# ur-whitelab/hoomd-tf

Hardware: AMD Instinct MI355X
Metric: MD steps/sec + achieved HBM GB/s, 131072 particles NN=128 (131k-particle box of the BASELINE metric) (higher is better)
Workload: dtype f32

## Files before the change

### hoomd_tf_amd/csrc/standin.hip

```cpp
#include <cstdlib>
#include <unordered_map>

#include "htf_common.h"
#include "box_math.h"
#include "htf_standin.h"
#include "standin_gate.h"
#include "key_sort.h"

namespace htf {

thread_local Gate g_gate = {nullptr, 0.f};

template <typename T>
__global__ __launch_bounds__(256) void nve_step_kernel(typename Vec4<T>::type *__restrict__ pos,
                                                       typename Vec4<T>::type *__restrict__ vel,
                                                       const typename Vec4<T>::type *__restrict__ force,
                                                       unsigned N, T dt, SBox<T> b) {
    unsigned i = blockIdx.x * blockDim.x + threadIdx.x;
    if (i >= N) return;
    auto p = pos[i];
    auto v = vel[i];
    nve_advance<T>(p, v, force[i], dt, b);
    pos[i] = p;
    vel[i] = v;
// ... 62 lines not shown
    for (unsigned m = 0; m < mirror.n; ++m) {
        const unsigned *src = (const unsigned *)mirror.src[m];
        unsigned *dst = (unsigned *)mirror.dst[m];
        for (unsigned w = threadIdx.x; w < mirror.words[m]; w += blockDim.x) dst[w] = __builtin_nontemporal_load(src + w);
    }
    __threadfence_system();
    __syncthreads();
    if (threadIdx.x == 0) {
        const float worst = __uint_as_float(atomicExch(work, 0u));
        const unsigned cycle = __float_as_uint(out[1]) + 1u;
        out[0] = worst;
        out[1] = __uint_as_float(cycle);
        work[1] = 0u;
        if (h_out != nullptr) {
            h_out[0] = worst;
            __threadfence_system();
            *(volatile unsigned *)(h_out + 1) = cycle;
        }
    }
}

template <typename T>
__device__ __forceinline__ int cell_coord(T x, T lo, T Linv, int n) {
    int c = (int)floor((x - lo) * Linv * (T)n);
    return c < 0 ? 0 : (c >= n ? n - 1 : c);
}

template <typename T>
__global__ __launch_bounds__(256) void cell_index_kernel(const typename Vec4<T>::type *__restrict__ pos, unsigned Ntot,
                                                         SBox<T> b, int nx, int ny, int nz,
                                                         unsigned *__restrict__ cell_of, Gate gate) {
    if (gate.closed()) return;
    unsigned i = blockIdx.x * blockDim.x + threadIdx.x;
    if (i >= Ntot) return;
    auto p = pos[i];
    if (is_inert(p.x)) {
        cell_of[i] = kDeadCell;
        return;
    }
    int cx = cell_coord<T>(p.x, b.lo[0], b.Linv[0], nx);
    int cy = cell_coord<T>(p.y, b.lo[1], b.Linv[1], ny);
    int cz = cell_coord<T>(p.z, b.lo[2], b.Linv[2], nz);
    cell_of[i] = (unsigned)((cz * ny + cy) * nx + cx);
}

constexpr unsigned kTagSide = 1u << 31;
constexpr unsigned kRangeWrapShift = 28u, kRangeLenMask = (1u << kRangeWrapShift) - 1u;
struct RangesArgs {
    int nx, ny, nz, wx, wy, wz, px, py, pz;
    const unsigned *cell_start;
    uint4 *table;
    unsigned *max_neigh;
};
__device__ __forceinline__ void cell_ranges_body(const unsigned t, const RangesArgs &a) {
    const int nx = a.nx, ny = a.ny, nz = a.nz, wx = a.wx, wy = a.wy, wz = a.wz, px = a.px, py = a.py, pz = a.pz;
    const unsigned *__restrict__ cell_start = a.cell_start;
    uint4 *__restrict__ table = a.table;
    unsigned *__restrict__ max_neigh = a.max_neigh;
    const int nrow = (2 * wy + 1) * (2 * wz + 1);
    if (t == 0) *max_neigh = 0u;
    const unsigned ncell = (unsigned)(nx * ny * nz);
    if (t >= ncell * (unsigned)nrow) return;
    const int c = (int)(t / nrow), r = (int)(t % nrow);
    const int cx = c % nx, cy = (c / nx) % ny, cz = c / (nx * ny);
    const int dz = r / (2 * wy + 1) - wz, dy = r % (2 * wy + 1) - wy;
    int a0 = cx - wx, a1 = cx + wx, b0 = 0, b1 = -1;
    if (a0 < 0) {
        if (px) { b0 = nx + a0; b1 = nx - 1; }
        a0 = 0;
    } else if (a1 >= nx) {
        if (px) { b0 = 0; b1 = a1 - nx; }
        a1 = nx - 1;
    }
    int ay = cy + dy, az = cz + dz;
    bool skip = false;
    unsigned wrap_y = 0u, wrap_z = 0u;
    if (ay < 0) { skip |= !py; ay += ny; wrap_y = 1u; } else if (ay >= ny) { skip |= !py; ay -= ny; wrap_y = 2u; }
    if (az < 0) { skip |= !pz; az += nz; wrap_z = 1u; } else if (az >= nz) { skip |= !pz; az -= nz; wrap_z = 2u; }
    uint4 o = make_uint4(0u, 0u, 0u, 0u);
    if (!skip) {
        const unsigned rowbase = (unsigned)((az * ny + ay) * nx);
        o.x = cell_start[rowbase + a0];
        o.y = (cell_start[rowbase + a1 + 1] - o.x) | (wrap_y << kRangeWrapShift) | (wrap_z << (kRangeWrapShift + 2));
        if (b1 >= b0) {
            o.z = cell_start[rowbase + b0];
            o.w = (cell_start[rowbase + b1 + 1] - o.z) | ((b0 == 0 ? 2u : 1u) << kRangeWrapShift);
        }
    }
    table[t] = o;
}
__global__ __launch_bounds__(256) void cell_ranges_kernel(RangesArgs a, Gate gate) {
    if (gate.closed()) return;
    cell_ranges_body(blockIdx.x * blockDim.x + threadIdx.x, a);
}

template <typename T, int G, bool SHIFT>
__global__ __launch_bounds__(256) void build_nlist_kernel(const typename Vec4<T>::type *__restrict__ pos,
                                                          const typename Vec4<T>::type *__restrict__ pos_sorted,
                                                          unsigned N, SBox<T> b, T rl2, int nx, int ny, int nz,
                                                          int wx, int wy, int wz,
                                                          const unsigned *__restrict__ cell_start, unsigned pitch,
                                                          int type_split,
                                                          unsigned *__restrict__ n_neigh, unsigned *__restrict__ head_list,
                                                          unsigned *__restrict__ nlist, unsigned *__restrict__ max_neigh,
                                                          const uint4 *__restrict__ ranges, Gate gate) {
    if (gate.closed()) return;
    const unsigned lane = threadIdx.x & 63u, g = lane % G, sub = lane / G;
    const unsigned i = ((blockIdx.x * blockDim.x + threadIdx.x) >> 6) * (64 / G) + sub;
    const bool in_range = i < N;
    const auto pi = pos[in_range ? i : 0];
    const bool active = in_range && !is_inert(pi.x);
    const int cx = cell_coord<T>(pi.x, b.lo[0], b.Linv[0], nx);
    const int cy = cell_coord<T>(pi.y, b.lo[1], b.Linv[1], ny);
    const int cz = cell_coord<T>(pi.z, b.lo[2], b.Linv[2], nz);
    const bool side_i = type_split >= 0 && scalar_as_int(pi.w) >= type_split;
    unsigned count = 0;
    unsigned *row = nlist + (size_t)(active ? i : 0) * pitch;
    const int nrow = (2 * wy + 1) * (2 * wz + 1);
    const uint4 *mine = ranges + (size_t)((cz * ny + cy) * nx + cx) * nrow;
    uint4 rg_next = active ? mine[0] : make_uint4(0u, 0u, 0u, 0u);
    for (int r = 0; r < nrow; ++r) {
        const uint4 rg = rg_next;
        if (r + 1 < nrow) rg_next = active ? mine[r + 1] : make_uint4(0u, 0u, 0u, 0u);
        T piy = pi.y, piz = pi.z, six = (T)0;
        if (SHIFT) {
            const unsigned wy_ = (rg.y >> kRangeWrapShift) & 3u, wz_ = rg.y >> (kRangeWrapShift + 2), wx_ = rg.w >> kRangeWrapShift;
            piy += wy_ == 1u ? b.L[1] : (wy_ == 2u ? -b.L[1] : (T)0);
            piz += wz_ == 1u ? b.L[2] : (wz_ == 2u ? -b.L[2] : (T)0);
            six = wx_ == 1u ? b.L[0] : -b.L[0];
        }
#pragma unroll
        for (int part = 0; part < 2; ++part) {
            const unsigned beg = part ? rg.z : rg.x, len = (part ? rg.w : rg.y) & kRangeLenMask;
            const T pix = (SHIFT && part) ? pi.x + six : pi.x;
// ... 127 lines not shown
#pragma unroll
            for (unsigned step = 32u; step != 0u; step >>= 1) {
                const unsigned t = at + step;
                at = bperm_u(t, start) <= q ? t : at;
            }
            const bool valid = q < total;
            const unsigned src = bperm_u(at, beg) + (q - bperm_u(at, start));
            V4 pk;
            pk.x = pk.y = pk.z = (T)0;
            set_tag(pk.w, ~0u);
            if (valid) pk = pos_sorted[src];
            if (any_shift) {
                pk.x -= bperm_t(at, shx);
                pk.y -= bperm_t(at, shy);
                pk.z -= bperm_t(at, shz);
            }
            const unsigned tag = (unsigned)scalar_as_int(pk.w);
            const unsigned k = tag & ~kTagSide;
            const unsigned long long vmask = ballot64(valid);
#pragma unroll
            for (int p = 0; p < kCellBatch; ++p) {
                const unsigned i = tag_p[p] & ~kTagSide;
                if (i >= N) continue;
                T ddx = pk.x - px[p], ddy = pk.y - py[p], ddz = pk.z - pz[p];
                if (!SHIFT) {
                    ddx = mimg<T>(ddx, b.L[0], b.Linv[0], b.periodic[0]);
                    ddy = mimg<T>(ddy, b.L[1], b.Linv[1], b.periodic[1]);
                    ddz = mimg<T>(ddz, b.L[2], b.Linv[2], b.periodic[2]);
                }
                unsigned long long hits = vmask & ballot64(k != i) & ballot64(ddx * ddx + ddy * ddy + ddz * ddz <= rl2);
                if (type_split >= 0) {
                    asm volatile("" ::: "memory");
                    hits &= ballot64(((tag ^ tag_p[p]) & kTagSide) == 0u);
                }
                const unsigned rank = __builtin_amdgcn_mbcnt_hi((unsigned)(hits >> 32), __builtin_amdgcn_mbcnt_lo((unsigned)hits, count[p]));
                if (inverse_ballot64(hits) && rank < pitch) nlist[row_p[p] + rank] = k;
                count[p] += (unsigned)__builtin_popcountll(hits);
            }
        }
        unsigned cnt = 0u;
#pragma unroll
        for (int p = 0; p < kCellBatch; ++p) cnt = lane == (unsigned)p ? count[p] : cnt;
        if (lane < np) {
            const unsigned i = my_tag & ~kTagSide;
            if (i < N) {
                n_neigh[i] = cnt < pitch ? cnt : pitch;
                head_list[i] = i * pitch;
                if (cnt > *(volatile unsigned *)max_neigh) atomicMax(max_neigh, cnt);
            }
        }
    }
}

}

using namespace htf;

extern "C" int htfs_nve_step(void *d_pos, void *d_vel, const void *d_force, int dtype, unsigned N, double dt,
                             const htf_box *box, htf_stream stream) {
    HTF_REQUIRE(d_pos && d_vel && d_force && box, "htfs_nve_step: null pointer");
    if (N == 0) return HTF_OK;
    unsigned grid = (N + 255) / 256;
    if (dtype == HTF_F32)
        hipLaunchKernelGGL((nve_step_kernel<float>), dim3(grid), dim3(256), 0, (hipStream_t)stream, (float4 *)d_pos, (float4 *)d_vel, (const float4 *)d_force, N, (float)dt, make_sbox<float>(box));
    else
        hipLaunchKernelGGL((nve_step_kernel<double>), dim3(grid), dim3(256), 0, (hipStream_t)stream, (double4 *)d_pos, (double4 *)d_vel, (const double4 *)d_force, N, dt, make_sbox<double>(box));
    return check_launch("nve_step_kernel");
}

extern "C" int htfs_max_displacement2(const void *d_pos, const void *d_ref, int dtype, unsigned N, const htf_box *box,
                                      float *d_out, htf_stream stream) {
    HTF_REQUIRE(d_pos && d_ref && box && d_out, "htfs_max_displacement2: null pointer");
    if (N == 0) return HTF_OK;
    unsigned grid = (N + 1023) / 1024;
    if (dtype == HTF_F32)
        hipLaunchKernelGGL((max_disp_kernel<float>), dim3(grid), dim3(1024), 0, (hipStream_t)stream, (const float4 *)d_pos, (const float4 *)d_ref, N, make_sbox<float>(box), d_out);
    else
        hipLaunchKernelGGL((max_disp_kernel<double>), dim3(grid), dim3(1024), 0, (hipStream_t)stream, (const double4 *)d_pos, (const double4 *)d_ref, N, make_sbox<double>(box), d_out);
    return check_launch("max_disp_kernel");
}

extern "C" int htfs_check_displacement2(const void *d_pos, const void *d_ref, int dtype, unsigned N, const htf_box *box,
                                        unsigned *d_work, float *d_out, float *h_out, const htfs_mirror *mirror, htf_stream stream) {
    using namespace htf;
    HTF_REQUIRE(d_pos && d_ref && box && d_work && d_out, "htfs_check_displacement2: null pointer");
    HTF_REQUIRE(N > 0, "htfs_check_displacement2: no rows");
    htfs_mirror mr = {};
    if (mirror != nullptr) {
        mr = *mirror;
        HTF_REQUIRE(mr.n <= HTFS_MIRROR_MAX, "htfs_check_displacement2: %u mirrors (at most %d)", mr.n, HTFS_MIRROR_MAX);
        for (unsigned m = 0; m < mr.n; ++m)
            HTF_REQUIRE(mr.src[m] && mr.dst[m] && ((uintptr_t)mr.src[m] & 3) == 0 && ((uintptr_t)mr.dst[m] & 3) == 0,
                        "htfs_check_displacement2: mirror %u: null or unaligned pointer", m);
    }
    unsigned grid = (N + 1023) / 1024;
    if (dtype == HTF_F32)
        hipLaunchKernelGGL((check_disp_kernel<float>), dim3(grid), dim3(1024), 0, (hipStream_t)stream, (const float4 *)d_pos, (const float4 *)d_ref, N, make_sbox<float>(box), d_work, d_out, h_out, mr);
    else
        hipLaunchKernelGGL((check_disp_kernel<double>), dim3(grid), dim3(1024), 0, (hipStream_t)stream, (const double4 *)d_pos, (const double4 *)d_ref, N, make_sbox<double>(box), d_work, d_out, h_out, mr);
    return check_launch("check_disp_kernel");
}

namespace htf {
struct Reimage {
    double L[3], c[3];
};
// ... 89 lines not shown
    for (unsigned i = 0; i < kScanPer; ++i) c[i] = first + i < ncell ? count[first + i] : 0u;
    unsigned sum = 0;
#pragma unroll
    for (unsigned i = 0; i < kScanPer; ++i) sum += c[i];
    unsigned incl = sum;
#pragma unroll
    for (unsigned off = 1; off < 64; off <<= 1) {
        const unsigned v = (unsigned)__shfl_up((int)incl, off);
        if (lane >= off) incl += v;
    }
    if (lane == 63) s_wave[wave] = incl;
    __syncthreads();
    unsigned before = 0, total = 0, carry = 0;
#pragma unroll
    for (unsigned w = 0; w < kScanThreads / 64; ++w) {
        const unsigned v = s_wave[w];
        before += w < wave ? v : 0u;
        total += v;
        carry += s_carry[w];
    }
    unsigned run = carry + before + (incl - sum);
#pragma unroll
    for (unsigned i = 0; i < kScanPer; ++i)
        if (first + i < ncell) {
            start[first + i] = run;
            cursor[first + i] = run;
            run += c[i];
        }
    if (blockIdx.x == gridDim.x - 1 && t == 0) start[ncell] = carry + total;
}

__global__ __launch_bounds__(256) void cell_scatter_kernel(const unsigned *__restrict__ cell_of, unsigned n,
                                                           unsigned *__restrict__ cursor, unsigned *__restrict__ order, Gate gate) {
    if (gate.closed()) return;
    const unsigned i = blockIdx.x * blockDim.x + threadIdx.x;
    if (i < n && cell_of[i] != kDeadCell) order[atomicAdd(&cursor[cell_of[i]], 1u)] = i;
}

__global__ __launch_bounds__(256) void cell_order_kernel(const unsigned *__restrict__ start, unsigned ncell,
                                                         unsigned *__restrict__ order, unsigned *__restrict__ count, Gate gate) {
    if (gate.closed()) return;
    const unsigned c = blockIdx.x * blockDim.x + threadIdx.x;
    if (c >= ncell) return;
    count[c] = 0u;
    const unsigned b = start[c], e = start[c + 1];
    for (unsigned i = b + 1; i < e; ++i) {
        const unsigned v = order[i];
        unsigned j = i;
        while (j > b && order[j - 1] > v) {
            order[j] = order[j - 1];
            --j;
        }
        order[j] = v;
    }
}
}

static int zero_counts_if_needed(unsigned *count, unsigned ncell, hipStream_t s) {
    static thread_local std::unordered_map<const void *, unsigned> zeroed_for;
    HTF_REQUIRE(((uintptr_t)count & 15) == 0, "binning scratch must be 16-byte aligned (cell_scan_kernel reads it with 16-byte loads)");
    auto it = zeroed_for.find(count);
    if (!g_gate.disp2 || it == zeroed_for.end() || it->second != ncell) {
        HTF_CHECK_HIP(hipMemsetAsync(count, 0, (size_t)ncell * sizeof(unsigned), s));
        zeroed_for[count] = ncell;
    }
    return HTF_OK;
}

extern "C" int htfs_cell_sort(const unsigned *d_cell_of, unsigned Ntot, unsigned ncell, unsigned *d_scratch,
                              unsigned *d_cell_start, unsigned *d_order, htf_stream stream) {
    using namespace htf;
    HTF_REQUIRE(d_cell_of && d_scratch && d_cell_start && d_order, "htfs_cell_sort: null pointer");
    HTF_REQUIRE(ncell > 0, "htfs_cell_sort: no cells");
    hipStream_t s = (hipStream_t)stream;
    unsigned *count = d_scratch, *cursor = d_scratch + ncell;
    if (int rc = zero_counts_if_needed(count, ncell, s)) return rc;
    if (Ntot) hipLaunchKernelGGL(cell_count_kernel, dim3((Ntot + 255) / 256), dim3(256), 0, s, d_cell_of, Ntot, count, g_gate);
    hipLaunchKernelGGL(cell_scan_kernel, dim3((ncell + kScanChunk - 1) / kScanChunk), dim3(kScanThreads), 0, s, count, ncell, d_cell_start, cursor, g_gate);
    if (Ntot) hipLaunchKernelGGL(cell_scatter_kernel, dim3((Ntot + 255) / 256), dim3(256), 0, s, d_cell_of, Ntot, cursor, d_order, g_gate);
    hipLaunchKernelGGL(cell_order_kernel, dim3((ncell + 255) / 256), dim3(256), 0, s, d_cell_start, ncell, d_order, count, g_gate);
    return check_launch("htfs_cell_sort");
}

static int gather4(void *d_dest, const void *d_src, const int *d_order, int dtype, unsigned n, bool tag, int type_split,
                   htf_stream stream, const unsigned *d_n_live = nullptr) {
    using namespace htf;
    HTF_REQUIRE(d_dest && d_src && d_order, "htfs_gather4: null pointer");
    HTF_REQUIRE(!tag || n <= kTagSide, "htfs_gather4_tagged: %u particles do not fit the 31-bit tag", n);
    if (n == 0) return HTF_OK;
    const dim3 grid((n + 255) / 256), block(256);
    hipStream_t s = (hipStream_t)stream;
    if (dtype == HTF_F32) {
        if (tag) hipLaunchKernelGGL((gather4_kernel<float4, true>), grid, block, 0, s, (float4 *)d_dest, (const float4 *)d_src, d_order, n, type_split, g_gate, d_n_live);
        else hipLaunchKernelGGL((gather4_kernel<float4, false>), grid, block, 0, s, (float4 *)d_dest, (const float4 *)d_src, d_order, n, type_split, g_gate, d_n_live);
    } else {
        if (tag) hipLaunchKernelGGL((gather4_kernel<double4, true>), grid, block, 0, s, (double4 *)d_dest, (const double4 *)d_src, d_order, n, type_split, g_gate, d_n_live);
        else hipLaunchKernelGGL((gather4_kernel<double4, false>), grid, block, 0, s, (double4 *)d_dest, (const double4 *)d_src, d_order, n, type_split, g_gate, d_n_live);
    }
    return check_launch("gather4_kernel");
}

extern "C" int htfs_gather4(void *d_dest, const void *d_src, const int *d_order, int dtype, unsigned n, htf_stream stream) {
    return gather4(d_dest, d_src, d_order, dtype, n, false, -1, stream);
}

extern "C" int htfs_gather4_tagged(void *d_dest, const void *d_src, const int *d_order, int dtype, unsigned n, int type_split,
// ... 62 lines not shown
#pragma unroll 1
    while (seg + 1 < t.n && row >= t.cnt[seg]) {
        row -= t.cnt[seg];
        ++seg;
    }
    dst[(size_t)(t.dst[seg] + row) * row_words + col] = src[(size_t)(t.src[seg] + row) * row_words + col];
}

extern "C" int htfs_segment_copy(void *d_dst, const void *d_src, unsigned row_bytes, unsigned n_segments,
                                 const unsigned *src_start, const unsigned *dst_start, const unsigned *count, htf_stream stream) {
    HTF_REQUIRE(d_dst && d_src && src_start && dst_start && count, "htfs_segment_copy: null pointer");
    HTF_REQUIRE(n_segments >= 1 && n_segments <= HTFS_MAX_SEGMENTS && row_bytes % 4 == 0 && row_bytes > 0,
                "htfs_segment_copy: need 1..%d segments of whole 32-bit words", HTFS_MAX_SEGMENTS);
    SegTable t;
    t.n = 0;
    unsigned total = 0;
    for (unsigned s = 0; s < n_segments; ++s) {
        if (count[s] == 0) continue;
        t.src[t.n] = src_start[s];
        t.dst[t.n] = dst_start[s];
        t.cnt[t.n] = count[s];
        total += count[s];
        ++t.n;
    }
    if (total == 0) return HTF_OK;
    const unsigned words = row_bytes / 4;
    const unsigned grid = (unsigned)(((size_t)total * words + 255) / 256);
    hipLaunchKernelGGL(segment_copy_kernel, dim3(grid), dim3(256), 0, (hipStream_t)stream, (unsigned *)d_dst, (const unsigned *)d_src,
                       words, t, total);
    return check_launch("segment_copy_kernel");
}

extern "C" int htfs_cell_index(const void *d_pos, int dtype, unsigned Ntot, const htf_box *box, const int *ncell3,
                               unsigned *d_cell_of, htf_stream stream) {
    HTF_REQUIRE(d_pos && box && ncell3 && d_cell_of, "htfs_cell_index: null pointer");
    if (Ntot == 0) return HTF_OK;
    unsigned grid = (Ntot + 255) / 256;
    if (dtype == HTF_F32)
        hipLaunchKernelGGL((cell_index_kernel<float>), dim3(grid), dim3(256), 0, (hipStream_t)stream, (const float4 *)d_pos, Ntot, make_sbox<float>(box), ncell3[0], ncell3[1], ncell3[2], d_cell_of, g_gate);
    else
        hipLaunchKernelGGL((cell_index_kernel<double>), dim3(grid), dim3(256), 0, (hipStream_t)stream, (const double4 *)d_pos, Ntot, make_sbox<double>(box), ncell3[0], ncell3[1], ncell3[2], d_cell_of, g_gate);
    return check_launch("cell_index_kernel");
}

struct FinishArgs {
    void *pos_sorted;
    const int *order;
    unsigned n;
    void *ref;
    unsigned n_ref;
    unsigned *counter;
    htf::Reimage im;
};

static int build_nlist_impl(const void *d_pos, const void *d_pos_sorted, int dtype, unsigned N, unsigned Ntot,
                            const htf_box *box, double r_list, const int *ncell3, const int *stencil3,
                            const unsigned *d_cell_start, unsigned pitch, int type_split,
                            unsigned *d_n_neigh, unsigned *d_head_list, unsigned *d_nlist, unsigned *d_max_neigh,
                            void *d_ranges_v, htf_stream stream, const FinishArgs *fin) {
    (void)Ntot;
    HTF_REQUIRE(d_pos && d_pos_sorted && box && ncell3 && stencil3 && d_cell_start && d_n_neigh && d_head_list && d_nlist && d_max_neigh,
                "htfs_build_nlist: null pointer");
    HTF_REQUIRE(pitch > 0, "htfs_build_nlist: pitch must be > 0");
    for (int d = 0; d < 3; ++d) {
        const double w = (box->hi[d] - box->lo[d]) / ncell3[d];
        const int sw = stencil3[d];
        HTF_REQUIRE((sw == 0 && ncell3[d] == 1) || (sw >= 1 && sw <= 2 && ncell3[d] >= 2 * sw + 1 && w * sw >= r_list * (1.0 - 1e-12)),
                    "htfs_build_nlist: along %d need 1 cell, or >= 2w+1 cells with w cells spanning r_list (got %d cells of %g, stencil %d, r_list %g)",
                    d, ncell3[d], w, sw, r_list);
    }
    if (N == 0) return HTF_OK;
    const unsigned ncell = (unsigned)(ncell3[0] * ncell3[1] * ncell3[2]);
    const unsigned nrow = (unsigned)((2 * stencil3[1] + 1) * (2 * stencil3[2] + 1));
    HTF_REQUIRE(d_ranges_v && ((uintptr_t)d_ranges_v & 15) == 0, "htfs_build_nlist: d_ranges must be a 16-byte aligned table of 4 * ncell * rows words");
    uint4 *d_ranges = (uint4 *)d_ranges_v;
    const RangesArgs ra = {ncell3[0], ncell3[1], ncell3[2], stencil3[0], stencil3[1], stencil3[2], (int)box->periodic[0],
                           (int)box->periodic[1], (int)box->periodic[2], d_cell_start, d_ranges, d_max_neigh};
    const unsigned nb_ranges = (ncell * nrow + 255) / 256;
    if (fin == nullptr) {
        hipLaunchKernelGGL(cell_ranges_kernel, dim3(nb_ranges), dim3(256), 0, (hipStream_t)stream, ra, g_gate);
    } else {
        const unsigned nb = nb_ranges + (fin->n + 255) / 256 + (fin->n == 0 ? 1u : 0u);
        if (dtype == HTF_F32)
            hipLaunchKernelGGL((bins_finish_kernel<float4>), dim3(nb), dim3(256), 0, (hipStream_t)stream, ra, nb_ranges, (float4 *)fin->pos_sorted,
                               (const float4 *)d_pos, fin->order, fin->n, type_split, (float4 *)fin->ref, fin->n_ref, fin->counter, fin->im, g_gate);
        else
            hipLaunchKernelGGL((bins_finish_kernel<double4>), dim3(nb), dim3(256), 0, (hipStream_t)stream, ra, nb_ranges, (double4 *)fin->pos_sorted,
                               (const double4 *)d_pos, fin->order, fin->n, type_split, (double4 *)fin->ref, fin->n_ref, fin->counter, fin->im, g_gate);
    }
    const bool fine = stencil3[0] == 2 || stencil3[1] == 2 || stencil3[2] == 2;
#define HTFS_NL(T, V4, G)                                                                                              \
    if (shift) HTFS_NL_(T, V4, G, true); else HTFS_NL_(T, V4, G, false)
#define HTFS_NL_(T, V4, G, S)                                                                                          \
    hipLaunchKernelGGL((build_nlist_kernel<T, G, S>), dim3((N + 4 * (64 / G) - 1) / (4 * (64 / G))), dim3(256), 0, (hipStream_t)stream, \
                       (const V4 *)d_pos, (const V4 *)d_pos_sorted, N, make_sbox<T>(box), (T)(r_list * r_list), ncell3[0],  \
                       ncell3[1], ncell3[2], stencil3[0], stencil3[1], stencil3[2], d_cell_start, pitch,      \
                       type_split, d_n_neigh, d_head_list, d_nlist, d_max_neigh, (const uint4 *)d_ranges, g_gate)
#define HTFS_NLC(T, V4)                                                                                                \
    if (shift) HTFS_NLC_(T, V4, true); else HTFS_NLC_(T, V4, false)
#define HTFS_NLC_(T, V4, S)                                                                                            \
    hipLaunchKernelGGL((build_nlist_cells_kernel<T, S>), dim3((ncell * cell_split + 3) / 4), dim3(256), 0, (hipStream_t)stream, \
                       (const V4 *)d_pos_sorted, N, make_sbox<T>(box), (T)(r_list * r_list), ncell, (int)nrow, d_cell_start, pitch, \
                       type_split, d_n_neigh, d_head_list, d_nlist, d_max_neigh, (const uint4 *)d_ranges, cell_split, g_gate)
    bool shift = true;
    for (int d = 0; d < 3; ++d) shift = shift && (!box->periodic[d] || ncell3[d] >= 7);
#ifdef HTF_AB_VARIANTS
    static const bool per_particle = std::getenv("HTFS_NLIST_PER_PARTICLE") != nullptr, per_cell = std::getenv("HTFS_NLIST_PER_CELL") != nullptr;
#else
    constexpr bool per_particle = false, per_cell = false;
#endif
    const bool reimaged = fin != nullptr && (fin->im.L[0] > 0.0 || fin->im.L[1] > 0.0 || fin->im.L[2] > 0.0);
    const bool by_cell = per_cell || reimaged || (!per_particle && ncell >= 1024u);
    const unsigned cell_split = ncell <= 12288u ? 2u : 1u;
    if (by_cell) {
        if (dtype == HTF_F32) { HTFS_NLC(float, float4); } else { HTFS_NLC(double, double4); }
    } else if (dtype == HTF_F32) {
        if (fine) { HTFS_NL(float, float4, 8); } else { HTFS_NL(float, float4, 16); }
    } else {
        if (fine) { HTFS_NL(double, double4, 8); } else { HTFS_NL(double, double4, 16); }
    }
#undef HTFS_NL
#undef HTFS_NL_
#undef HTFS_NLC
#undef HTFS_NLC_
    return check_launch("build_nlist_kernel");
}

extern "C" int htfs_build_nlist(const void *d_pos, const void *d_pos_sorted, int dtype, unsigned N, unsigned Ntot,
                                const htf_box *box, double r_list, const int *ncell3, const int *stencil3,
                                const unsigned *d_cell_start, unsigned pitch, int type_split,
                                unsigned *d_n_neigh, unsigned *d_head_list, unsigned *d_nlist, unsigned *d_max_neigh,
                                void *d_ranges, htf_stream stream) {
    return build_nlist_impl(d_pos, d_pos_sorted, dtype, N, Ntot, box, r_list, ncell3, stencil3, d_cell_start, pitch, type_split, d_n_neigh,
                            d_head_list, d_nlist, d_max_neigh, d_ranges, stream, nullptr);
}

static int rebuild_nlist_impl(const void *d_pos, int dtype, unsigned N, unsigned Ntot, const htf_box *box, double r_list, const int *ncell3,
                              const int *stencil3, unsigned *d_cell_of, unsigned *d_scratch, unsigned *d_cell_start,
                              unsigned *d_order, void *d_pos_sorted, unsigned pitch, int type_split, unsigned *d_n_neigh,
                              unsigned *d_head_list, unsigned *d_nlist, unsigned *d_max_neigh, void *d_ref,
                              unsigned *d_counter, void *d_ranges, htf_stream stream, bool scratch_clean = false,
                              const double *image_L = nullptr) {
    using namespace htf;
    HTF_REQUIRE(d_pos && box && ncell3 && stencil3 && d_cell_of && d_scratch && d_cell_start && d_order && d_pos_sorted,
                "htfs_rebuild_nlist: null pointer");
    HTF_REQUIRE(Ntot >= N, "htfs_rebuild_nlist: Ntot %u < N %u", Ntot, N);
    if (N == 0) return HTF_OK;
    const unsigned ncell = (unsigned)(ncell3[0] * ncell3[1] * ncell3[2]);
    HTF_REQUIRE(ncell > 0, "htfs_rebuild_nlist: no cells");
    hipStream_t s = (hipStream_t)stream;
    unsigned *count = d_scratch, *cursor = d_scratch + ncell;
    if (!scratch_clean)
        if (int rc = zero_counts_if_needed(count, ncell, s)) return rc;
    const unsigned grid = (Ntot + 255) / 256;
    Reimage im = {};
    for (int d = 0; d < 3; ++d) {
        im.L[d] = image_L != nullptr && !box->periodic[d] ? image_L[d] : 0.0;
        im.c[d] = 0.5 * (box->lo[d] + box->hi[d]);
        HTF_REQUIRE(im.L[d] == 0.0 || im.L[d] >= box->hi[d] - box->lo[d], "htfs_rebuild_nlist_ghosts: image length %g along axis %d is shorter than the grid", im.L[d], d);
    }
    if (dtype == HTF_F32)
        hipLaunchKernelGGL((cell_index_count_kernel<float>), dim3(grid), dim3(256), 0, s, (const float4 *)d_pos, Ntot, make_sbox<float>(box),
                           ncell3[0], ncell3[1], ncell3[2], d_cell_of, count, im, g_gate);
    else
        hipLaunchKernelGGL((cell_index_count_kernel<double>), dim3(grid), dim3(256), 0, s, (const double4 *)d_pos, Ntot, make_sbox<double>(box),
                           ncell3[0], ncell3[1], ncell3[2], d_cell_of, count, im, g_gate);
    hipLaunchKernelGGL(cell_scan_kernel, dim3((ncell + kScanChunk - 1) / kScanChunk), dim3(kScanThreads), 0, s, count, ncell, d_cell_start, cursor, g_gate);
    hipLaunchKernelGGL(cell_scatter_kernel, dim3(grid), dim3(256), 0, s, d_cell_of, Ntot, cursor, d_order, g_gate);
    hipLaunchKernelGGL(cell_order_kernel, dim3((ncell + 255) / 256), dim3(256), 0, s, d_cell_start, ncell, d_order, count, g_gate);
    const FinishArgs fin = {d_pos_sorted, (const int *)d_order, Ntot, d_ref, N, d_counter, im};
    return build_nlist_impl(d_pos, d_pos_sorted, dtype, N, Ntot, box, r_list, ncell3, stencil3, d_cell_start, pitch, type_split, d_n_neigh,
                            d_head_list, d_nlist, d_max_neigh, d_ranges, stream, &fin);
}

extern "C" int htfs_rebuild_nlist(const void *d_pos, int dtype, unsigned N, const htf_box *box, double r_list, const int *ncell3,
                                  const int *stencil3, unsigned *d_cell_of, unsigned *d_scratch, unsigned *d_cell_start,
                                  unsigned *d_order, void *d_pos_sorted, unsigned pitch, int type_split, unsigned *d_n_neigh,
                                  unsigned *d_head_list, unsigned *d_nlist, unsigned *d_max_neigh, void *d_ref,
                                  unsigned *d_counter, void *d_ranges, htf_stream stream) {
    return rebuild_nlist_impl(d_pos, dtype, N, N, box, r_list, ncell3, stencil3, d_cell_of, d_scratch, d_cell_start, d_order, d_pos_sorted,
                              pitch, type_split, d_n_neigh, d_head_list, d_nlist, d_max_neigh, d_ref, d_counter, d_ranges, stream);
}

extern "C" int htfs_rebuild_nlist_ghosts(const void *d_pos, int dtype, unsigned N, unsigned Ntot, const htf_box *box, double r_list,
                                         const int *ncell3, const int *stencil3, unsigned *d_cell_of, unsigned *d_scratch,
                                         unsigned *d_cell_start, unsigned *d_order, void *d_pos_sorted, unsigned pitch, int type_split,
                                         unsigned *d_n_neigh, unsigned *d_head_list, unsigned *d_nlist, unsigned *d_max_neigh, void *d_ref,
                                         unsigned *d_counter, void *d_ranges, int scratch_clean, const double *image_L, htf_stream stream) {
    return rebuild_nlist_impl(d_pos, dtype, N, Ntot, box, r_list, ncell3, stencil3, d_cell_of, d_scratch, d_cell_start, d_order, d_pos_sorted,
                              pitch, type_split, d_n_neigh, d_head_list, d_nlist, d_max_neigh, d_ref, d_counter, d_ranges, stream,
                              scratch_clean != 0, image_L);
}

extern "C" int htfs_check_rebuild_nlist(const void *d_pos, int dtype, unsigned N, const htf_box *box, double r_list, const int *ncell3,
                                        const int *stencil3, unsigned *d_cell_of, unsigned *d_scratch, unsigned *d_cell_start,
                                        unsigned *d_order, void *d_pos_sorted, unsigned pitch, int type_split, unsigned *d_n_neigh,
                                        unsigned *d_head_list, unsigned *d_nlist, unsigned *d_stat2, void *d_ref, float *d_disp2,
                                        double threshold2, unsigned *h_stat2, void *d_ranges, htf_stream stream) {
    HTF_REQUIRE(d_ref && d_disp2 && d_stat2, "htfs_check_rebuild_nlist: null pointer");
    if (N == 0) return HTF_OK;
    HTF_CHECK_HIP(hipMemsetAsync(d_disp2, 0, sizeof(float), (hipStream_t)stream));
    int rc = htfs_max_displacement2(d_pos, d_ref, dtype, N, box, d_disp2, stream);
    if (rc != HTF_OK) return rc;
    rc = htfs_set_gate(d_disp2, threshold2);
    if (rc != HTF_OK) return rc;
    rc = htfs_rebuild_nlist(d_pos, dtype, N, box, r_list, ncell3, stencil3, d_cell_of, d_scratch, d_cell_start, d_order, d_pos_sorted, pitch,
                            type_split, d_n_neigh, d_head_list, d_nlist, d_stat2, d_ref, d_stat2 + 1, d_ranges, stream);
    (void)htfs_set_gate(nullptr, 0.0);
    if (rc != HTF_OK) return rc;
    if (h_stat2 != nullptr)
        HTF_CHECK_HIP(hipMemcpyAsync(h_stat2, d_stat2, 2 * sizeof(unsigned), hipMemcpyDeviceToHost, (hipStream_t)stream));
    return HTF_OK;
}
// ... 29 lines not shown
```

Baseline: 13460.

## Replace six-kernel neighbor-list rebuild with three-kernel bin-count, place, search pipeline

The rebuild path now bins particles into fixed-capacity per-cell slot arrays using atomics. A single place kernel computes cell starts via a block-local prefix sum, orders each cell's members by rank and writes the sorted, reimaged positions. A new search kernel computes the stencil row ranges inside each wave (prefix sum plus binary search over the rows) instead of reading a precomputed range table. This removes the separate scan, scatter, insertion-sort and ranges kernels and their launches. The cost is a slow fallback scan over all particles when a cell overflows its cap, and reuse of the ranges buffer as slot storage.

```diff
diff --git a/hoomd_tf_amd/csrc/standin.hip b/hoomd_tf_amd/csrc/standin.hip
--- a/hoomd_tf_amd/csrc/standin.hip
+++ b/hoomd_tf_amd/csrc/standin.hip
@@ -138,34 +138,48 @@
     uint4 *table;
     unsigned *max_neigh;
 };
+struct RowSpan {
+    int a0, a1, b0, b1;
+    unsigned rowbase, wrap_y, wrap_z;
+    bool skip;
+};
+__device__ __forceinline__ RowSpan row_span(const RangesArgs &a, int c, int r) {
+    const int nx = a.nx, ny = a.ny, nz = a.nz, wx = a.wx, wy = a.wy, wz = a.wz, px = a.px, py = a.py, pz = a.pz;
+    const int cx = c % nx, cy = (c / nx) % ny, cz = c / (nx * ny);
+    const int dw = 2 * wy + 1, q = (r >= dw) + (r >= 2 * dw) + (r >= 3 * dw) + (r >= 4 * dw);
+    const int dz = q - wz, dy = r - q * dw - wy;
+    RowSpan s;
+    s.a0 = cx - wx, s.a1 = cx + wx, s.b0 = 0, s.b1 = -1;
+    if (s.a0 < 0) {
+        if (px) { s.b0 = nx + s.a0; s.b1 = nx - 1; }
+        s.a0 = 0;
+    } else if (s.a1 >= nx) {
+        if (px) { s.b0 = 0; s.b1 = s.a1 - nx; }
+        s.a1 = nx - 1;
+    }
+    int ay = cy + dy, az = cz + dz;
+    s.skip = false;
+    s.wrap_y = 0u, s.wrap_z = 0u;
+    if (ay < 0) { s.skip |= !py; ay += ny; s.wrap_y = 1u; } else if (ay >= ny) { s.skip |= !py; ay -= ny; s.wrap_y = 2u; }
+    if (az < 0) { s.skip |= !pz; az += nz; s.wrap_z = 1u; } else if (az >= nz) { s.skip |= !pz; az -= nz; s.wrap_z = 2u; }
+    s.rowbase = (unsigned)((az * ny + ay) * nx);
+    return s;
+}
 __device__ __forceinline__ void cell_ranges_body(const unsigned t, const RangesArgs &a) {
-    const int nx = a.nx, ny = a.ny, nz = a.nz, wx = a.wx, wy = a.wy, wz = a.wz, px = a.px, py = a.py, pz = a.pz;
     const unsigned *__restrict__ cell_start = a.cell_start;
     uint4 *__restrict__ table = a.table;
     unsigned *__restrict__ max_neigh = a.max_neigh;
-    const int nrow = (2 * wy + 1) * (2 * wz + 1);
+    const int nrow = (2 * a.wy + 1) * (2 * a.wz + 1);
     if (t == 0) *max_neigh = 0u;
-    const unsigned ncell = (unsigned)(nx * ny * nz);
+    const unsigned ncell = (unsigned)(a.nx * a.ny * a.nz);
     if (t >= ncell * (unsigned)nrow) return;
     const int c = (int)(t / nrow), r = (int)(t % nrow);
-    const int cx = c % nx, cy = (c / nx) % ny, cz = c / (nx * ny);
-    const int dz = r / (2 * wy + 1) - wz, dy = r % (2 * wy + 1) - wy;
-    int a0 = cx - wx, a1 = cx + wx, b0 = 0, b1 = -1;
-    if (a0 < 0) {
-        if (px) { b0 = nx + a0; b1 = nx - 1; }
-        a0 = 0;
-    } else if (a1 >= nx) {
-        if (px) { b0 = 0; b1 = a1 - nx; }
-        a1 = nx - 1;
-    }
-    int ay = cy + dy, az = cz + dz;
-    bool skip = false;
-    unsigned wrap_y = 0u, wrap_z = 0u;
-    if (ay < 0) { skip |= !py; ay += ny; wrap_y = 1u; } else if (ay >= ny) { skip |= !py; ay -= ny; wrap_y = 2u; }
-    if (az < 0) { skip |= !pz; az += nz; wrap_z = 1u; } else if (az >= nz) { skip |= !pz; az -= nz; wrap_z = 2u; }
+    const RowSpan s = row_span(a, c, r);
+    const int a0 = s.a0, a1 = s.a1, b0 = s.b0, b1 = s.b1;
+    const unsigned wrap_y = s.wrap_y, wrap_z = s.wrap_z;
     uint4 o = make_uint4(0u, 0u, 0u, 0u);
-    if (!skip) {
-        const unsigned rowbase = (unsigned)((az * ny + ay) * nx);
+    if (!s.skip) {
+        const unsigned rowbase = s.rowbase;
         o.x = cell_start[rowbase + a0];
         o.y = (cell_start[rowbase + a1 + 1] - o.x) | (wrap_y << kRangeWrapShift) | (wrap_z << (kRangeWrapShift + 2));
         if (b1 >= b0) {
@@ -399,6 +413,148 @@
     }
 }
 
+constexpr int kSearchTripsDefault = 1;
+template <typename T, bool SHIFT, int kSearchTrips>
+__global__ __launch_bounds__(256) void search_cells_kernel(const typename Vec4<T>::type *__restrict__ pos_sorted, unsigned N, SBox<T> b,
+                                                           T rl2, RangesArgs ra, unsigned pitch, int type_split,
+                                                           unsigned *__restrict__ n_neigh, unsigned *__restrict__ head_list,
+                                                           unsigned *__restrict__ nlist, unsigned *__restrict__ max_neigh, unsigned split,
+                                                           unsigned *__restrict__ bin_count, Gate gate) {
+    if (gate.closed()) return;
+    using V4 = typename Vec4<T>::type;
+    const unsigned lane = threadIdx.x & 63u;
+    const unsigned *__restrict__ cell_start = ra.cell_start;
+    const unsigned ncell = (unsigned)(ra.nx * ra.ny * ra.nz);
+    const int nrow = (2 * ra.wy + 1) * (2 * ra.wz + 1);
+    const unsigned wv = __builtin_amdgcn_readfirstlane((blockIdx.x * blockDim.x + threadIdx.x) >> 6);
+    const unsigned c = wv / split, b0 = wv % split;
+    if (c >= ncell) return;
+    if (b0 == 0u && lane == 0u) bin_count[c] = 0u;
+    const unsigned p_begin = cell_start[c], p_end = cell_start[c + 1];
+    if (p_begin + b0 * (unsigned)kCellBatch >= p_end) return;
+
+    unsigned beg = 0u, len = 0u;
+    T shx = (T)0, shy = (T)0, shz = (T)0;
+    if (lane < 2u * (unsigned)nrow) {
+        const RowSpan s = row_span(ra, (int)c, (int)(lane >> 1));
+        const bool wrapped = (lane & 1u) != 0u;
+        const int lo = wrapped ? s.b0 : s.a0, hi = wrapped ? s.b1 : s.a1;
+        if (!s.skip && hi >= lo) {
+            beg = cell_start[s.rowbase + lo];
+            len = cell_start[s.rowbase + hi + 1] - beg;
+        }
+        if (SHIFT) {
+            shy = s.wrap_y == 1u ? b.L[1] : (s.wrap_y == 2u ? -b.L[1] : (T)0);
+            shz = s.wrap_z == 1u ? b.L[2] : (s.wrap_z == 2u ? -b.L[2] : (T)0);
+            shx = !wrapped ? (T)0 : (s.b0 == 0 ? -b.L[0] : b.L[0]);
+        }
+    }
+    if (p_end - p_begin <= 64u) {
+        const bool local = lane < p_end - p_begin && ((unsigned)scalar_as_int(pos_sorted[p_begin + lane].w) & ~kTagSide) < N;
+        if (ballot64(local) == 0ull) return;
+    }
+    unsigned incl = len;
+#pragma unroll
+    for (unsigned d = 1; d < 64u; d <<= 1) {
+        const unsigned up = bperm_u(lane >= d ? lane - d : lane, incl);
+        incl += lane >= d ? up : 0u;
+    }
+    const unsigned start = incl - len;
+    const unsigned total = (unsigned)__builtin_amdgcn_readlane((int)incl, 63);
+    const bool any_shift = SHIFT && ballot64(len != 0u && (shx != (T)0 || shy != (T)0 || shz != (T)0)) != 0ull;
+
+    for (unsigned pb = p_begin + b0 * (unsigned)kCellBatch; pb < p_end; pb += split * (unsigned)kCellBatch) {
+        const unsigned np = min(p_end - pb, (unsigned)kCellBatch);
+        V4 me;
+        me.x = me.y = me.z = (T)0;
+        set_tag(me.w, ~0u);
+        if (lane < np) me = pos_sorted[pb + lane];
+        const unsigned my_tag = (unsigned)scalar_as_int(me.w);
+        if (ballot64(lane < np && (my_tag & ~kTagSide) < N) == 0ull) continue;
+        unsigned tag_p[kCellBatch], count[kCellBatch];
+        T px[kCellBatch], py[kCellBatch], pz[kCellBatch];
+        unsigned row_p[kCellBatch];
+#pragma unroll
+        for (int p = 0; p < kCellBatch; ++p) {
+            tag_p[p] = ~0u;
+            px[p] = py[p] = pz[p] = (T)0;
+            count[p] = 0u;
+            row_p[p] = 0u;
+            if ((unsigned)p < np) {
+                tag_p[p] = (unsigned)__builtin_amdgcn_readlane((int)my_tag, p);
+                px[p] = in_vgpr(bcast_lane_t(me.x, p));
+                py[p] = in_vgpr(bcast_lane_t(me.y, p));
+                pz[p] = in_vgpr(bcast_lane_t(me.z, p));
+                row_p[p] = (tag_p[p] & ~kTagSide) * pitch;
+            }
+        }
+        for (unsigned q0 = 0; q0 < total; q0 += 64u * kSearchTrips) {
+            V4 pk[kSearchTrips];
+            unsigned at[kSearchTrips];
+#pragma unroll
+            for (int u = 0; u < kSearchTrips; ++u) {
+                pk[u].x = pk[u].y = pk[u].z = (T)0;
+                set_tag(pk[u].w, ~0u);
+                at[u] = 0u;
+                if (q0 + 64u * u >= total) continue;
+                const unsigned q = q0 + 64u * u + lane;
+                unsigned a_ = 0u;
+#pragma unroll
+                for (unsigned step = 32u; step != 0u; step >>= 1) {
+                    const unsigned t = a_ + step;
+                    a_ = bperm_u(t, start) <= q ? t : a_;
+                }
+                at[u] = a_;
+                const unsigned src = bperm_u(a_, beg) + (q - bperm_u(a_, start));
+                if (q < total) pk[u] = pos_sorted[src];
+            }
+#pragma unroll
+            for (int u = 0; u < kSearchTrips; ++u) {
+                if (q0 + 64u * u >= total) break;
+                V4 cand = pk[u];
+                if (any_shift) {
+                    cand.x -= bperm_t(at[u], shx);
+                    cand.y -= bperm_t(at[u], shy);
+                    cand.z -= bperm_t(at[u], shz);
+                }
+                const unsigned tag = (unsigned)scalar_as_int(cand.w);
+                const unsigned k = tag & ~kTagSide;
+                const unsigned long long vmask = ballot64(q0 + 64u * u + lane < total);
+#pragma unroll
+                for (int p = 0; p < kCellBatch; ++p) {
+                    const unsigned i = tag_p[p] & ~kTagSide;
+                    if (i >= N) continue;
+                    T ddx = cand.x - px[p], ddy = cand.y - py[p], ddz = cand.z - pz[p];
+                    if (!SHIFT) {
+                        ddx = mimg<T>(ddx, b.L[0], b.Linv[0], b.periodic[0]);
+                        ddy = mimg<T>(ddy, b.L[1], b.Linv[1], b.periodic[1]);
+                        ddz = mimg<T>(ddz, b.L[2], b.Linv[2], b.periodic[2]);
+                    }
+                    unsigned long long hits = vmask & ballot64(k != i) & ballot64(ddx * ddx + ddy * ddy + ddz * ddz <= rl2);
+                    if (type_split >= 0) {
+                        asm volatile("" ::: "memory");
+                        hits &= ballot64(((tag ^ tag_p[p]) & kTagSide) == 0u);
+                    }
+                    const unsigned rank = __builtin_amdgcn_mbcnt_hi((unsigned)(hits >> 32), __builtin_amdgcn_mbcnt_lo((unsigned)hits, count[p]));
+                    if (inverse_ballot64(hits) && rank < pitch) nlist[row_p[p] + rank] = k;
+                    count[p] += (unsigned)__builtin_popcountll(hits);
+                }
+            }
+        }
+        unsigned cnt = 0u;
+#pragma unroll
+        for (int p = 0; p < kCellBatch; ++p) cnt = lane == (unsigned)p ? count[p] : cnt;
+        if (lane < np) {
+            const unsigned i = my_tag & ~kTagSide;
+            if (i < N) {
+                n_neigh[i] = cnt < pitch ? cnt : pitch;
+                head_list[i] = i * pitch;
+                if (cnt > *(volatile unsigned *)max_neigh) atomicMax(max_neigh, cnt);
+            }
+        }
+    }
+}
+
 }
 
 using namespace htf;
@@ -594,6 +750,115 @@
             --j;
         }
         order[j] = v;
+    }
+}
+
+constexpr unsigned kBinLanes = 8, kBinCells = 256 / kBinLanes;
+
+template <typename T>
+__global__ __launch_bounds__(256) void bin_count_kernel(const typename Vec4<T>::type *__restrict__ pos, unsigned Ntot, SBox<T> b,
+                                                        int nx, int ny, int nz, unsigned *__restrict__ cell_of,
+                                                        unsigned *__restrict__ count, unsigned *__restrict__ slots, unsigned cap,
+                                                        Reimage im, Gate gate) {
+    if (gate.closed()) return;
+    const unsigned i = blockIdx.x * blockDim.x + threadIdx.x;
+    if (i >= Ntot) return;
+    const auto p = pos[i];
+    if (is_inert(p.x)) {
+        cell_of[i] = kDeadCell;
+        return;
+    }
+    const int cx = cell_coord<T>(reimage1(p.x, im.L[0], im.c[0]), b.lo[0], b.Linv[0], nx);
+    const int cy = cell_coord<T>(reimage1(p.y, im.L[1], im.c[1]), b.lo[1], b.Linv[1], ny);
+    const int cz = cell_coord<T>(reimage1(p.z, im.L[2], im.c[2]), b.lo[2], b.Linv[2], nz);
+    const unsigned c = (unsigned)((cz * ny + cy) * nx + cx);
+    cell_of[i] = c;
+    const unsigned slot = atomicAdd(&count[c], 1u);
+    if (slot < cap) slots[(size_t)c * cap + slot] = i;
+}
+
+template <typename V>
+__global__ __launch_bounds__(256) void bin_place_kernel(unsigned ncell, unsigned Ntot, const unsigned *__restrict__ cell_of,
+                                                        const unsigned *__restrict__ count, const unsigned *__restrict__ slots,
+                                                        unsigned cap, unsigned *__restrict__ cell_start, unsigned *__restrict__ order,
+                                                        V *__restrict__ dest, const V *__restrict__ src, int type_split, V *__restrict__ ref,
+                                                        unsigned n_ref, unsigned *__restrict__ counter, unsigned *__restrict__ max_neigh,
+                                                        Reimage im, Gate gate) {
+    if (gate.closed()) return;
+    __shared__ unsigned s_before[4], s_cnt[kBinCells], s_start[kBinCells];
+    const unsigned t = threadIdx.x, lane = t & 63u, g = t % kBinLanes, cl = t / kBinLanes;
+    const unsigned c = blockIdx.x * kBinCells + cl;
+    unsigned before = 0u;
+    {
+        const uint4 *q = reinterpret_cast<const uint4 *>(count);
+        const unsigned nq = blockIdx.x * (kBinCells / 4u);
+        for (unsigned j0 = 0; j0 < nq; j0 += 8u * blockDim.x) {
+            uint4 v[8];
+#pragma unroll
+            for (unsigned u = 0; u < 8u; ++u) {
+                const unsigned j = j0 + u * blockDim.x + t;
+                v[u] = j < nq ? q[j] : make_uint4(0u, 0u, 0u, 0u);
+            }
+#pragma unroll
+            for (unsigned u = 0; u < 8u; ++u) before += (v[u].x + v[u].y) + (v[u].z + v[u].w);
+        }
+    }
+    before = group_sum_u<64>(before);
+    if (lane == 0u) s_before[t >> 6] = before;
+    const unsigned cnt = c < ncell ? count[c] : 0u;
+    if (g == 0u) s_cnt[cl] = cnt;
+    if (t == 0u && blockIdx.x == 0u) {
+        if (counter != nullptr) *counter += 1u;
+        *max_neigh = 0u;
+    }
+    __syncthreads();
+    if (t < kBinCells) {
+        const unsigned v = s_cnt[t];
+        unsigned incl = v;
+#pragma unroll
+        for (unsigned off = 1; off < kBinCells; off <<= 1) {
+            const unsigned up = (unsigned)__shfl_up((int)incl, off, kBinCells);
+            if (t >= off) incl += up;
+        }
+        const unsigned base = (s_before[0] + s_before[1]) + (s_before[2] + s_before[3]);
+        s_start[t] = base + incl - v;
+        if (t == kBinCells - 1u && blockIdx.x == gridDim.x - 1u) cell_start[ncell] = base + incl;
+    }
+    __syncthreads();
+    const unsigned first = s_start[cl];
+    if (g == 0u && c < ncell) cell_start[c] = first;
+    auto place = [&](unsigned k, unsigned d) {
+        order[d] = k;
+        V p = src[k];
+        if (ref != nullptr && k < n_ref) ref[k] = p;
+        p.x = reimage1(p.x, im.L[0], im.c[0]);
+        p.y = reimage1(p.y, im.L[1], im.c[1]);
+        p.z = reimage1(p.z, im.L[2], im.c[2]);
+        set_tag(p.w, k | ((type_split >= 0 && scalar_as_int(p.w) >= type_split) ? kTagSide : 0u));
+        dest[d] = p;
+    };
+    const bool fits = cnt <= cap;
+    const unsigned *mine = slots + (size_t)(c < ncell ? c : 0u) * cap;
+    for (unsigned k0 = 0; ballot64(fits && k0 < cnt) != 0ull; k0 += kBinLanes) {
+        const bool have = fits && k0 + g < cnt;
+        const unsigned me = have ? mine[k0 + g] : ~0u;
+        unsigned rank = 0u;
+        for (unsigned j0 = 0; ballot64(fits && j0 < cnt) != 0ull; j0 += kBinLanes) {
+            const unsigned o = fits && j0 + g < cnt ? mine[j0 + g] : ~0u;
+#pragma unroll
+            for (unsigned j = 0; j < kBinLanes; ++j) rank += (unsigned)__shfl((int)o, (int)j, (int)kBinLanes) < me ? 1u : 0u;
+        }
+        if (have) place(me, first + rank);
+    }
+    if (ballot64(!fits) != 0ull) {
+        unsigned done = 0u;
+        for (unsigned j0 = 0; j0 < Ntot; j0 += kBinLanes) {
+            const unsigned j = j0 + g;
+            const bool hit = !fits && j < Ntot && cell_of[j] == c;
+            const unsigned m = (unsigned)(ballot64(hit) >> (lane & ~(kBinLanes - 1u))) & ((1u << kBinLanes) - 1u);
+            if (hit) place(j, first + done + (unsigned)__popc(m & ((1u << g) - 1u)));
+            done += (unsigned)__popc(m);
+        }
     }
 }
 }
@@ -762,6 +1027,17 @@
     unsigned *counter;
     htf::Reimage im;
 };
+
+static bool search_by_cell(unsigned ncell, const htf::Reimage *im) {
+#ifdef HTF_AB_VARIANTS
+    static const bool per_particle = std::getenv("HTFS_NLIST_PER_PARTICLE") != nullptr, per_cell = std::getenv("HTFS_NLIST_PER_CELL") != nullptr;
+#else
+    constexpr bool per_particle = false, per_cell = false;
+#endif
+    const bool reimaged = im != nullptr && (im->L[0] > 0.0 || im->L[1] > 0.0 || im->L[2] > 0.0);
+    return per_cell || reimaged || (!per_particle && ncell >= 1024u);
+}
+static unsigned search_cell_split(unsigned ncell) { return ncell <= 12288u ? 2u : 1u; }
 
 static int build_nlist_impl(const void *d_pos, const void *d_pos_sorted, int dtype, unsigned N, unsigned Ntot,
                             const htf_box *box, double r_list, const int *ncell3, const int *stencil3,
@@ -814,14 +1090,8 @@
                        type_split, d_n_neigh, d_head_list, d_nlist, d_max_neigh, (const uint4 *)d_ranges, cell_split, g_gate)
     bool shift = true;
     for (int d = 0; d < 3; ++d) shift = shift && (!box->periodic[d] || ncell3[d] >= 7);
-#ifdef HTF_AB_VARIANTS
-    static const bool per_particle = std::getenv("HTFS_NLIST_PER_PARTICLE") != nullptr, per_cell = std::getenv("HTFS_NLIST_PER_CELL") != nullptr;
-#else
-    constexpr bool per_particle = false, per_cell = false;
-#endif
-    const bool reimaged = fin != nullptr && (fin->im.L[0] > 0.0 || fin->im.L[1] > 0.0 || fin->im.L[2] > 0.0);
-    const bool by_cell = per_cell || reimaged || (!per_particle && ncell >= 1024u);
-    const unsigned cell_split = ncell <= 12288u ? 2u : 1u;
+    const bool by_cell = search_by_cell(ncell, fin != nullptr ? &fin->im : nullptr);
+    const unsigned cell_split = search_cell_split(ncell);
     if (by_cell) {
         if (dtype == HTF_F32) { HTFS_NLC(float, float4); } else { HTFS_NLC(double, double4); }
     } else if (dtype == HTF_F32) {
@@ -869,6 +1139,63 @@
         im.c[d] = 0.5 * (box->lo[d] + box->hi[d]);
         HTF_REQUIRE(im.L[d] == 0.0 || im.L[d] >= box->hi[d] - box->lo[d], "htfs_rebuild_nlist_ghosts: image length %g along axis %d is shorter than the grid", im.L[d], d);
     }
+#ifdef HTF_AB_VARIANTS
+    static const bool three = std::getenv("HTFS_REBUILD_LEGACY") == nullptr;
+#else
+    constexpr bool three = true;
+#endif
+    if (three && ncell >= 2u && search_by_cell(ncell, &im)) {
+        HTF_REQUIRE(d_ranges && ((uintptr_t)d_ranges & 15) == 0 && d_n_neigh && d_head_list && d_nlist && d_max_neigh,
+                    "htfs_rebuild_nlist: null pointer");
+        for (int d = 0; d < 3; ++d) {
+            const double w = (box->hi[d] - box->lo[d]) / ncell3[d];
+            const int sw = stencil3[d];
+            HTF_REQUIRE((sw == 0 && ncell3[d] == 1) || (sw >= 1 && sw <= 2 && ncell3[d] >= 2 * sw + 1 && w * sw >= r_list * (1.0 - 1e-12)),
+                        "htfs_build_nlist: along %d need 1 cell, or >= 2w+1 cells with w cells spanning r_list (got %d cells of %g, stencil %d, r_list %g)",
+                        d, ncell3[d], w, sw, r_list);
+        }
+        HTF_REQUIRE(pitch > 0, "htfs_build_nlist: pitch must be > 0");
+        HTF_REQUIRE(Ntot <= kTagSide, "htfs_rebuild_nlist: %u particles do not fit the 31-bit tag", Ntot);
+        const unsigned nrow = (unsigned)((2 * stencil3[1] + 1) * (2 * stencil3[2] + 1));
+        unsigned *slots = (unsigned *)d_ranges;
+        const unsigned cap = 4u * nrow;
+        const RangesArgs ra = {ncell3[0], ncell3[1], ncell3[2], stencil3[0], stencil3[1], stencil3[2], (int)box->periodic[0],
+                               (int)box->periodic[1], (int)box->periodic[2], d_cell_start, nullptr, d_max_neigh};
+        const dim3 place_grid((ncell + kBinCells - 1) / kBinCells), search_grid((ncell * search_cell_split(ncell) + 3) / 4);
+        bool shift = true;
+        for (int d = 0; d < 3; ++d) shift = shift && (!box->periodic[d] || ncell3[d] >= 7);
+#ifdef HTF_AB_VARIANTS
+        static const int trips = std::getenv("HTFS_SEARCH_TRIPS") != nullptr ? std::atoi(std::getenv("HTFS_SEARCH_TRIPS")) : kSearchTripsDefault;
+#else
+        constexpr int trips = kSearchTripsDefault;
+#endif
+#define HTFS_SEARCH3(T, V4, S, U)                                                                                                     \
+    hipLaunchKernelGGL((search_cells_kernel<T, S, U>), search_grid, dim3(256), 0, s, (const V4 *)d_pos_sorted, N, make_sbox<T>(box),  \
+                       (T)(r_list * r_list), ra, pitch, type_split, d_n_neigh, d_head_list, d_nlist, d_max_neigh,                     \
+                       search_cell_split(ncell), count, g_gate)
+#define HTFS_REBUILD3(T, V4)                                                                                                          \
+    do {                                                                                                                              \
+        hipLaunchKernelGGL((bin_count_kernel<T>), dim3(grid), dim3(256), 0, s, (const V4 *)d_pos, Ntot, make_sbox<T>(box), ncell3[0],  \
+                           ncell3[1], ncell3[2], d_cell_of, count, slots, cap, im, g_gate);                                           \
+        hipLaunchKernelGGL((bin_place_kernel<V4>), place_grid, dim3(256), 0, s, ncell, Ntot, d_cell_of, count, slots, cap,            \
+                           d_cell_start, d_order, (V4 *)d_pos_sorted, (const V4 *)d_pos, type_split, (V4 *)d_ref, N, d_counter,       \
+                           d_max_neigh, im, g_gate);                                                                                  \
+        if (shift) {                                                                                                                  \
+            if (trips == 1) HTFS_SEARCH3(T, V4, true, 1);                                                                             \
+            else if (trips == 2) HTFS_SEARCH3(T, V4, true, 2);                                                                        \
+            else HTFS_SEARCH3(T, V4, true, 4);                                                                                        \
+        } else {                                                                                                                      \
+            if (trips == 1) HTFS_SEARCH3(T, V4, false, 1);                                                                            \
+            else if (trips == 2) HTFS_SEARCH3(T, V4, false, 2);                                                                       \
+            else HTFS_SEARCH3(T, V4, false, 4);                                                                                       \
+        }                                                                                                                             \
+    } while (0)
+        if (dtype == HTF_F32) HTFS_REBUILD3(float, float4);
+        else HTFS_REBUILD3(double, double4);
+#undef HTFS_SEARCH3
+#undef HTFS_REBUILD3
+        return check_launch("htfs_rebuild_nlist");
+    }
     if (dtype == HTF_F32)
         hipLaunchKernelGGL((cell_index_count_kernel<float>), dim3(grid), dim3(256), 0, s, (const float4 *)d_pos, Ntot, make_sbox<float>(box),
                            ncell3[0], ncell3[1], ncell3[2], d_cell_of, count, im, g_gate);
```

Result: faster. 13880, median of 6 (+3.2%).
